# boguszjelinski/taxidispatcher

Hardware: AMD Instinct MI355X
Metric: NxN assignments/sec (higher is better)
Workload: dtype int32; 1 GPU; g1 N=16384: device cost write (4N^2 B) + exact assignment, total checked == optimum; n=16384, parallelism=single GPU

## Files before the change

taxidispatcher_amd/csrc/td_assign.hip:

```cpp
#include <dlfcn.h>
#include <limits.h>
#include <stdlib.h>

#include <type_traits>

#include "td_common.h"

using namespace td;

namespace {

template <typename CT>
struct Tr;
template <>
struct Tr<uint8_t> {
    using PT = int32_t;
    static constexpr int E = 16;
    static constexpr uint32_t SENT = 0xFFu;
    static constexpr int64_t LIMIT = 254;
    static constexpr int32_t BIG = 1 << 28;
    static constexpr int32_t KMAX = INT32_MAX;
};
template <>
struct Tr<uint16_t> {
// ... 100 lines not shown
int g_cgrid = 4;
int g_creg = 1;
int g_speculate = 1;
int g_sap8 = 1;
int g_psap8_batches = 1;
int g_psap8_grid = 64;
int g_warm_tie_div = 2;
int g_u16_redo_free = 64;
int g_wide_u16_n = 2048;
bool g_line = true;
int g_line_min_n = 2;
int g_psap_batches = 16;
int g_psap_min = 12;
int g_psap_cap = 4096;
int g_warm = 1;
int g_warm_div = 4;
int g_warm_theta = 2;
int g_warm_bits = 30;
int g_warm_groups = 32;
int g_warm_cut = 64;
int g_warm_min_range = 256;
int g_warm_minfree = 32;
int g_warm_min_n = 512;
int g_sapx = 1;
int g_sapx_min = 8;
int g_sapx_slim_chunks = INT_MAX;
int g_sapx_rows = 24;
int g_sap512 = 1;
int g_psap_worth = 4;
int g_bid0 = 1;
int g_defer_const = 1;
int g_shape = 1;
int g_shape_max_n = 1 << 20;
int g_narrow_price = 1;
long long g_np_plimit = NP_PLIMIT;
int g_fuse_t = 2;
int g_fuse_spec = 1;
int g_fused_rounds = 8;
int g_fuse_gen = 1;
int g_tick_rounds = 5;
int g_forest = 1;
int g_forest_min_n = 2048;
long long g_forest_w0 = 16;
long long g_forest_wx = 16;
int g_blocks = -1;
int g_blocks_min_n = 12288;
int g_zs_rounds = 4;
int g_zs_sep = 0;
int g_hop_passes = 2;
int g_hop_max_rows = HOP_FMAX;
int g_lazy_cc = 1;
int g_hop_global = 1;
int g_one_trip = 1;
int g_zs_global_rounds = 6;
int g_core = 1;
int g_core_k = 64;
int g_core_min_n = 8192;
int g_core_mode = 1;
double g_core_eps = 1.0;
int g_rand_test = 1;
int g_rand_div = 8192;
int g_rand_rounds = 48;
int g_rand_repeat = 1;
double g_rand_corr = 0.12;
int g_core_patience = 6;
int g_solver_eps = 0;
int g_eps_theta = 8;
long long g_eps0_mult = 4;
void read_tunables()
{
    static bool done = false;
    if (done) return;
    done = true;
    if (const char *e = getenv("TD_MAX_ROUNDS")) g_max_rounds = std::max(1, std::min(48, atoi(e)));
    if (const char *e = getenv("TD_TIE_EVICT")) g_tie_evict = atoi(e) != 0;
    if (const char *e = getenv("TD_LDS_ROUNDS")) g_lds_rounds = std::max(0, atoi(e));
    if (const char *e = getenv("TD_SAP8")) g_sap8 = atoi(e) != 0;
    if (const char *e = getenv("TD_ROW_LOOP")) g_row_loop = std::max(0, atoi(e));
    if (const char *e = getenv("TD_ROW_ROUNDS")) g_row_rounds = std::max(0, atoi(e));
    if (const char *e = getenv("TD_CGRID")) g_cgrid = std::max(1, atoi(e));
    if (const char *e = getenv("TD_CREG")) g_creg = atoi(e) != 0;
    if (const char *e = getenv("TD_PSAP")) g_psap_batches = std::max(0, std::min(64, atoi(e)));
    if (const char *e = getenv("TD_PSAP_MIN")) g_psap_min = std::max(1, atoi(e));
    if (const char *e = getenv("TD_PSAP_CAP")) g_psap_cap = std::max(0, atoi(e));
    if (const char *e = getenv("TD_SAP512")) g_sap512 = atoi(e) != 0;
    if (const char *e = getenv("TD_SAPX")) g_sapx = atoi(e) != 0;
    if (const char *e = getenv("TD_WARM")) g_warm = atoi(e) != 0;
    if (const char *e = getenv("TD_WARM_DIV")) g_warm_div = std::max(1, atoi(e));
    if (const char *e = getenv("TD_WARM_THETA")) g_warm_theta = std::max(2, atoi(e));
    if (const char *e = getenv("TD_WARM_BITS")) g_warm_bits = std::max(1, std::min(30, atoi(e)));
    if (const char *e = getenv("TD_WARM_GROUPS")) g_warm_groups = std::max(1, atoi(e));
    if (const char *e = getenv("TD_WARM_CUT")) g_warm_cut = std::max(0, atoi(e));
    if (const char *e = getenv("TD_WARM_MIN_RANGE")) g_warm_min_range = std::max(1, atoi(e));
    if (const char *e = getenv("TD_WARM_MINFREE")) g_warm_minfree = std::max(1, atoi(e));
    if (const char *e = getenv("TD_WARM_MIN_N")) g_warm_min_n = std::max(0, atoi(e));
    if (const char *e = getenv("TD_SAPX_MIN")) g_sapx_min = std::max(1, atoi(e));
    if (const char *e = getenv("TD_SAPX_SLIM")) g_sapx_slim_chunks = std::max(64, atoi(e));
    if (const char *e = getenv("TD_SAPX_ROWS")) g_sapx_rows = std::max(1, atoi(e));
    if (const char *e = getenv("TD_PSAP_WORTH")) g_psap_worth = std::max(1, atoi(e));
    if (const char *e = getenv("TD_SPECULATE")) g_speculate = atoi(e) != 0;
    if (const char *e = getenv("TD_LDS_GRID")) g_lds_grid = std::max(1, std::min(8, atoi(e)));
    if (const char *e = getenv("TD_NARROW_PRICE")) g_narrow_price = atoi(e) != 0;
    if (const char *e = getenv("TD_NP_PLIMIT")) g_np_plimit = std::max(1ll, std::min((long long)NP_PLIMIT, atoll(e)));
    if (const char *e = getenv("TD_FUSE_T")) g_fuse_t = std::max(0, std::min(2, atoi(e)));
    if (const char *e = getenv("TD_FUSE_SPEC")) g_fuse_spec = atoi(e) != 0;
    if (const char *e = getenv("TD_FUSED_ROUNDS")) g_fused_rounds = std::max(1, std::min(48, atoi(e)));
    if (const char *e = getenv("TD_FUSE_GEN")) g_fuse_gen = atoi(e) != 0;
    if (const char *e = getenv("TD_TICK_ROUNDS")) g_tick_rounds = std::max(1, std::min(48, atoi(e)));
    if (const char *e = getenv("TD_FOREST")) g_forest = atoi(e) != 0;
    if (const char *e = getenv("TD_FOREST_MIN_N")) g_forest_min_n = std::max(64, atoi(e));
    if (const char *e = getenv("TD_FOREST_W0")) g_forest_w0 = std::max(1ll, atoll(e));
    if (const char *e = getenv("TD_FOREST_WX")) g_forest_wx = std::max(0ll, atoll(e));
    if (const char *e = getenv("TD_SOLVER")) g_solver_eps = (strcmp(e, "eps") == 0);
    if (const char *e = getenv("TD_EPS0_MULT")) g_eps0_mult = std::max(0ll, atoll(e));
    if (const char *e = getenv("TD_EPS_THETA")) g_eps_theta = std::max(2, atoi(e));
    if (const char *e = getenv("TD_PSAP8")) g_psap8_batches = std::max(0, std::min(32, atoi(e)));
    if (const char *e = getenv("TD_DEFER_CONST")) g_defer_const = atoi(e) != 0;
    if (const char *e = getenv("TD_BID0")) g_bid0 = atoi(e) != 0;
    if (const char *e = getenv("TD_SHAPE")) g_shape = atoi(e) != 0;
    if (const char *e = getenv("TD_SHAPE_MAX_N")) g_shape_max_n = atoi(e);
    if (const char *e = getenv("TD_WIDE_U16_N")) g_wide_u16_n = std::max(0, atoi(e));
    if (const char *e = getenv("TD_U16_REDO_FREE")) g_u16_redo_free = std::max(0, atoi(e));
    if (const char *e = getenv("TD_WARM_TIE_DIV")) g_warm_tie_div = std::max(1, atoi(e));
    if (const char *e = getenv("TD_LINE")) g_line = atoi(e) != 0;
    if (const char *e = getenv("TD_LINE_MIN_N")) g_line_min_n = std::max(2, atoi(e));
    if (const char *e = getenv("TD_PSAP8_GRID")) g_psap8_grid = std::max(1, std::min(192, atoi(e)));
    if (const char *e = getenv("TD_CORE")) g_core = atoi(e) != 0;
    if (const char *e = getenv("TD_CORE_K")) g_core_k = std::max(2, std::min(200, atoi(e)));
    if (const char *e = getenv("TD_CORE_MIN_N")) g_core_min_n = std::max(256, atoi(e));
    if (const char *e = getenv("TD_CORE_MODE")) g_core_mode = atoi(e);
    if (const char *e = getenv("TD_CORE_EPS")) g_core_eps = atof(e);
    if (const char *e = getenv("TD_CORE_PATIENCE")) g_core_patience = std::max(1, atoi(e));
    if (const char *e = getenv("TD_RAND_TEST")) g_rand_test = atoi(e) != 0;
    if (const char *e = getenv("TD_RAND_DIV")) g_rand_div = std::max(1, atoi(e));
    if (const char *e = getenv("TD_RAND_ROUNDS")) g_rand_rounds = std::max(1, std::min(48, atoi(e)));
    if (const char *e = getenv("TD_RAND_CORR")) g_rand_corr = atof(e);
    if (const char *e = getenv("TD_RAND_REPEAT")) g_rand_repeat = std::max(1, atoi(e));
    if (const char *e = getenv("TD_BLOCKS")) g_blocks = std::max(-1, std::min(HOP_BMAX, atoi(e)));
    if (const char *e = getenv("TD_BLOCKS_MIN_N")) g_blocks_min_n = std::max(0, atoi(e));
    if (const char *e = getenv("TD_ZS_ROUNDS")) g_zs_rounds = std::max(0, std::min(32, atoi(e)));
    if (const char *e = getenv("TD_ZS_SEP")) g_zs_sep = atoi(e) != 0;
    if (const char *e = getenv("TD_HOP_PASSES")) g_hop_passes = std::max(0, std::min(8, atoi(e)));
    if (const char *e = getenv("TD_HOP_MAX_ROWS")) g_hop_max_rows = std::max(1, atoi(e));
    if (const char *e = getenv("TD_HOP_GLOBAL")) g_hop_global = atoi(e) != 0;
    if (const char *e = getenv("TD_ONE_TRIP")) g_one_trip = atoi(e) != 0;
    if (const char *e = getenv("TD_LAZY_CC")) g_lazy_cc = atoi(e) != 0;
    if (const char *e = getenv("TD_ZS_GLOBAL_ROUNDS")) g_zs_global_rounds = std::max(1, std::min(48, atoi(e)));
}

template <typename CT>
__device__ __forceinline__ void unpack(const uint4 &v, uint32_t *out);
template <>
__device__ __forceinline__ void unpack<uint8_t>(const uint4 &v, uint32_t *o)
{
    const uint32_t w[4] = {v.x, v.y, v.z, v.w};
#pragma unroll
    for (int k = 0; k < 4; k++) {
        o[4 * k + 0] = w[k] & 0xFFu;
        o[4 * k + 1] = (w[k] >> 8) & 0xFFu;
        o[4 * k + 2] = (w[k] >> 16) & 0xFFu;
        o[4 * k + 3] = w[k] >> 24;
    }
}
template <>
__device__ __forceinline__ void unpack<u8e>(const uint4 &v, uint32_t *o)
{
    const uint32_t w[4] = {v.x, v.y, v.z, v.w};
    const uint32_t esc = g_esc8;
#pragma unroll
    for (int k = 0; k < 4; k++) {
#pragma unroll
        for (int b = 0; b < 4; b++) {
            const uint32_t x = (w[k] >> (8 * b)) & 0xFFu;
            o[4 * k + b] = (x == U8E_ESC) ? esc : x;
        }
    }
}
template <>
__device__ __forceinline__ void unpack<uint16_t>(const uint4 &v, uint32_t *o)
{
    const uint32_t w[4] = {v.x, v.y, v.z, v.w};
#pragma unroll
    for (int k = 0; k < 4; k++) {
        o[2 * k + 0] = w[k] & 0xFFFFu;
        o[2 * k + 1] = w[k] >> 16;
    }
}
template <>
__device__ __forceinline__ void unpack<uint32_t>(const uint4 &v, uint32_t *o)
{
    o[0] = v.x;
    o[1] = v.y;
    o[2] = v.z;
    o[3] = v.w;
}
template <>
__device__ __forceinline__ void unpack<u32n>(const uint4 &v, uint32_t *o)
{
    o[0] = v.x;
// ... 2843 lines not shown
    using PT = typename Tr<CT>::PT;
    int rc;
    if ((rc = ensure(sv.esc, sizeof(unsigned long long) * 2 * (size_t)std::max(sv.nrows, 1)))) return rc;
    if ((rc = ensure(sv.hop, sizeof(HopCtl)))) return rc;
    if ((rc = ensure(sv.hoptab, sizeof(int) * (size_t)nb * HOP_FMAX * HOP_FMAX))) return rc;
    HopCtl *hc = (HopCtl *)sv.hop.p;
    int *frl = (int *)sv.list.p, *fcl = (int *)sv.pred.p;
    const int *ctl = (const int *)sv.misc.p;
    if (gate && nb != 1) return fail(TD_EINTERNAL, "a gated two-hop pass takes one block");
    k_hop_lists<<<nb, 1024, 0, c.stream>>>(rpb, ncols_blk, col_lo, (const int *)sv.r2c.p, (const int *)sv.owner.p, frl, fcl, hc, ctl,
                                           gate ? g_hop_max_rows : 0);
    if (raw) {
        if (!sv.d_cost || sv.n % 4) return fail(TD_EINVAL, "two-hop pass on the int32 matrix: no matrix, or n %% 4 != 0");
        k_hop_esc<CT, true><<<(sv.nrows + 3) / 4, 256, 0, c.stream>>>(sv.nrows, sv.n / 4, rpb, ncols_blk, col_lo, g_hop_max_rows,
                                                                      (const CT *)sv.d_cost, (const PT *)sv.price.p, (const int *)sv.r2c.p, fcl,
                                                                      hc, (unsigned long long *)sv.esc.p, ctl, (const int32_t *)sv.rowmin.p);
        k_hop_table<CT, true><<<nb * HOP_FMAX, 256, 0, c.stream>>>(sv.n, sv.nrows, sv.row0, sv.n / 4, rpb, ncols_blk, col_lo, g_hop_max_rows,
                                                                   window_zero ? 1 : 0, (const CT *)sv.d_cost, (const PT *)sv.price.p,
                                                                   (const int *)sv.owner.p, frl, hc, (const unsigned long long *)sv.esc.p,
                                                                   (int *)sv.hoptab.p, ctl, (const int32_t *)sv.rowmin.p);
    } else {
    k_hop_esc<CT><<<(sv.nrows + 3) / 4, 256, 0, c.stream>>>(sv.nrows, sv.nchunks, rpb, ncols_blk, col_lo, g_hop_max_rows, (const CT *)sv.cc.p,
                                                            (const PT *)sv.price.p, (const int *)sv.r2c.p, fcl, hc,
                                                            (unsigned long long *)sv.esc.p, ctl);
    k_hop_table<CT><<<nb * HOP_FMAX, 256, 0, c.stream>>>(sv.n, sv.nrows, sv.row0, sv.nchunks, rpb, ncols_blk, col_lo, g_hop_max_rows,
                                                         window_zero ? 1 : 0, (const CT *)sv.cc.p, (const PT *)sv.price.p,
                                                         (const int *)sv.owner.p, frl, hc, (const unsigned long long *)sv.esc.p,
                                                         (int *)sv.hoptab.p, ctl);
    }
    k_hop_match<PT><<<nb, HOP_FMAX, sizeof(uint32_t) * (size_t)((rpb + 31) / 32), c.stream>>>(
        sv.nrows, sv.row0, rpb, ncols_blk, col_lo, g_hop_max_rows, (PT *)sv.price.p, (int *)sv.owner.p, (int *)sv.r2c.p, ob, frl, fcl, hc,
        (const int *)sv.hoptab.p, (int *)sv.misc.p);
    TD_HIP(hipGetLastError());
    return TD_OK;
}

template <typename CT>
int sv_begin_t(Solver &sv);

int sv_phase_a(Solver &sv, int hop_passes)
{
    Ctx &c = ctx();
    const int n = sv.n, nrows = sv.nrows;
    const int rpb = n / sv.zs_V, nb = nrows / rpb;
    const int col_lo = (sv.row0 / rpb) * rpb, col_hi = col_lo + nb * rpb;
    int rc;
    if ((rc = ensure(sv.ob, (size_t)sv.npad + 64))) return rc;
    if (!sv.ob_clear) TD_HIP(hipMemsetAsync(sv.ob.p, 0, (size_t)sv.npad, c.stream));
    sv.ob_clear = false;
    ProfScope ps(TD_K_BID);
    int *ctl = (int *)sv.misc.p;
    const int ga = (col_hi - col_lo + 255) / 256;
    unsigned long long *bid = (unsigned long long *)sv.bid.p;
    auto assign = [&]() {
        k_zs_assign<<<ga, 256, 0, c.stream>>>(col_lo, col_hi, nrows, sv.row0, bid, (int32_t *)sv.price.p, (int *)sv.owner.p, (int *)sv.r2c.p,
                                              (uint8_t *)sv.ob.p, ctl);
    };
    if (sv.zs_round0) {
        if (!sv.began && (rc = sv_begin_t<uint8_t>(sv))) return rc;
        k_zs_bid<<<std::min(nrows, c.n_cu * 16), 256, 0, c.stream>>>(nrows, sv.row0, sv.nchunks, rpb, (const uint8_t *)sv.cc.p,
                                                                     (const uint8_t *)sv.ob.p, (const int *)sv.r2c.p, bid, ctl, 0, 0);
        sv.zs_round0 = false;
    }
    assign();
    for (int r = 1; r <= g_zs_rounds; r++) {
        k_zs_bid<<<std::min(nrows, c.n_cu * 16), 256, 0, c.stream>>>(nrows, sv.row0, sv.nchunks, rpb, (const uint8_t *)sv.cc.p,
                                                                     (const uint8_t *)sv.ob.p, (const int *)sv.r2c.p, bid, ctl, r, g_tie_evict);
        assign();
    }
    TD_HIP(hipGetLastError());
    for (int p = 0; p < hop_passes; p++)
        if ((rc = sv_hop_t<uint8_t>(sv, rpb, rpb, col_lo, nb, true, (uint8_t *)sv.ob.p))) return rc;
    if (getenv("TD_DEBUG") && hop_passes > 0) {
        HopCtl h;
        TD_HIP(hipMemcpyAsync(&h, sv.hop.p, sizeof(h), hipMemcpyDeviceToHost, c.stream));
        TD_HIP(hipStreamSynchronize(c.stream));
        fprintf(stderr, "[td] phase A: %d blocks of %d rows, %d local rounds; free rows / columns per block before the last two-hop pass:", nb, rpb, g_zs_rounds);
        for (int b = 0; b < nb; b++) fprintf(stderr, " %d/%d", h.nfr[b], h.nfc[b]);
        fprintf(stderr, " | matched %d, left %d\n", h.matched, h.left);
    }
    sv.zs_done = false;
    sv.bid0_done = false;
    sv.state_ready = true;
    return TD_OK;
}

template <typename CT>
int sv_begin_t(Solver &sv)
{
    Ctx &c = ctx();
    using PT = typename Tr<CT>::PT;
    const PT padkey = (PT)(Tr<CT>::BIG << 1) | (PT)1;
    k_init_state<PT><<<(std::max(sv.npad, (int)CTL_WORDS) + 255) / 256, 256, 0, c.stream>>>(
        sv.n, sv.npad, sv.nrows, (PT *)sv.price.p, padkey, (int *)sv.owner.p, (int *)sv.r2c.p,
        (unsigned long long *)sv.bid.p, (int *)sv.misc.p, sv.defer_const ? (const int *)sv.rconst.p : nullptr, sv.probe, 0, nullptr,
        g_one_trip ? (unsigned long long *)((char *)sv.misc.p + FIN_OFF) : nullptr);
    if (!g_one_trip) TD_HIP(hipMemsetAsync((char *)sv.misc.p + FIN_OFF, 0, 16, c.stream));
    TD_HIP(hipGetLastError());
    sv.began = true;
    return TD_OK;
}

template <typename CT>
int sv_bid_t(Solver &sv, int r, unsigned long long *keys)
{
    Ctx &c = ctx();
    using PT = typename Tr<CT>::PT;
    const int n = sv.n, nrows = sv.nrows;
    if (nrows == 0) return TD_OK;
    const size_t lds_prices = (size_t)sv.npad * sizeof(PT);
    const bool can_lds = lds_prices <= 128 * 1024 && n >= 2048 && nrows >= 1024;
    const int tie_evict = (r >= 1) ? g_tie_evict : 0;
    ProfScope ps(TD_K_BID);
    int *tied = (r == 0) ? (int *)sv.misc.p + CTL_TIED : nullptr;
    const bool sparse = sv.state_ready;
    if (can_lds && r < g_lds_rounds && !sparse) {
        if (lds_prices > 48 * 1024)
            (void)hipFuncSetAttribute((const void *)k_bid<CT, true>, hipFuncAttributeMaxDynamicSharedMemorySize, (int)lds_prices);
        const int grid = std::min((nrows + 15) / 16, c.n_cu * g_lds_grid);
        k_bid<CT, true><<<grid, 1024, lds_prices, c.stream>>>(n, nrows, sv.row0, sv.nchunks, (const CT *)sv.cc.p, (const PT *)sv.price.p,
                                                              (const int *)sv.r2c.p, keys, (const int *)sv.misc.p, r, tie_evict, 1, 0, tied);
    } else if (r >= g_row_rounds || sparse) {
        k_bid_row<CT><<<(r < g_row_loop && !sparse) ? nrows : std::min(nrows, c.n_cu * 8), 256, 0, c.stream>>>(n, nrows, sv.row0, sv.nchunks, (const CT *)sv.cc.p, (const PT *)sv.price.p,
                                                   (const int *)sv.r2c.p, keys, (const int *)sv.misc.p, r, tie_evict);
    } else {
// ... 1255 lines not shown
__global__ void k_state_import(int n, int world, int rps, int words, int own_rank, const int32_t *__restrict__ all,
                               int *__restrict__ owner, int32_t *__restrict__ pk, int *__restrict__ cmask, long long *__restrict__ summary)
{
    const int t = blockIdx.x * blockDim.x + threadIdx.x;
    if (t == 0) {
        long long fit = 1, ran = 1, left = 0, nconst = 0, range = 0;
        for (int r = 0; r < world; r++) {
            const int32_t *h = all + (size_t)r * words;
            fit = fit && h[0];
            ran = ran && h[1];
            left += h[2] >= 0 ? h[2] : n;
            nconst += h[3];
            const long long rg = (long long)(((unsigned long long)(uint32_t)h[5] << 32) | (uint32_t)h[4]);
            range = rg > range ? rg : range;
        }
        summary[0] = fit;
        summary[1] = ran;
        summary[2] = left;
        summary[3] = nconst;
        summary[4] = range;
        summary[5] = all[6];
    }
    if (t < n) {
        const int r = t / rps, k = t - r * rps;
        const int32_t *seg = all + (size_t)r * words;
        if (r != own_rank) {
            const int o = seg[16 + k];
            owner[t] = o;
            pk[t] = (pk[t] & ~1) | (o >= 0 ? 1 : 0);
        }
        cmask[t] = seg[16 + rps + k];
    }
}
}

extern "C" {
int td_shard_state_export(td_shard *s, int rows_per_shard, int fits, int32_t *seg)
{
    TD_REQUIRE_INIT();
    Ctx &c = ctx();
    if (!s || !seg || rows_per_shard < s->nrows) return fail(TD_EINVAL, "td_shard_state_export: bad arguments");
    if (!is_device_ptr(seg)) return fail(TD_EINVAL, "td_shard_state_export: the segment must be device memory");
    const bool ran = s->state_ready && s->bpc == 1 && s->zs_V > 0;
    int col_lo = 0;
    if (ran) col_lo = (s->row0 / (s->n / s->zs_V)) * (s->n / s->zs_V);
    ProfScope ps(TD_K_ASSIGN);
    k_state_export<<<(std::max(rows_per_shard, 16) + 255) / 256, 256, 0, c.stream>>>(
        s->nrows, rows_per_shard, col_lo, fits ? 1 : 0, ran ? 1 : 0, (const int *)s->owner.p, (const int *)s->rconst.p,
        ran ? (const HopCtl *)s->hop.p : nullptr, (const int *)s->misc.p, seg);
    TD_HIP(hipGetLastError());
    return TD_OK;
}

int td_shard_state_import(td_shard *s, int world, int rank, int rows_per_shard, const int32_t *all, int64_t *summary5)
{
    TD_REQUIRE_INIT();
    Ctx &c = ctx();
    if (!s || !all || !summary5 || world < 1 || rank < 0 || rank >= world) return fail(TD_EINVAL, "td_shard_state_import: bad arguments");
    if (!is_device_ptr(all)) return fail(TD_EINVAL, "td_shard_state_import: the segments must be device memory");
    if ((long long)rows_per_shard * world < s->n) return fail(TD_EINVAL, "td_shard_state_import: rows_per_shard * world < n");
    int rc;
    if ((rc = ensure(s->cmask, sizeof(int) * (size_t)(s->n + 16)))) return rc;
    long long *sum_dev = (long long *)((char *)s->misc.p + 2048);
    const int words = 16 + 2 * rows_per_shard;
    {
        ProfScope ps(TD_K_ASSIGN);
        k_state_import<<<(s->n + 255) / 256, 256, 0, c.stream>>>(s->n, world, rows_per_shard, words, rank, all, (int *)s->owner.p,
                                                            (int32_t *)s->price.p, (int *)s->cmask.p, sum_dev);
    }
    TD_HIP(hipGetLastError());
    TD_HIP(hipMemcpyAsync(c.pinned, sum_dev, 6 * sizeof(long long), hipMemcpyDeviceToHost, c.stream));
    TD_HIP(hipStreamSynchronize(c.stream));
    for (int k = 0; k < 6; k++) summary5[k] = ((const long long *)c.pinned)[k];
    s->have_cmask = true;
    s->defer_const = g_defer_const && !g_solver_eps;
    return TD_OK;
}

int td_shard_range(td_shard *s, int64_t *range)
{
    TD_REQUIRE_INIT();
    if (!s || !range) return fail(TD_EINVAL, "null argument");
    *range = s->range > 0 ? s->range : std::max<int64_t>(0, s->fit_bound);
    return TD_OK;
}

int td_shard_begin(td_shard *s, int64_t global_range)
{
    TD_REQUIRE_INIT();
    if (!s) return fail(TD_EINVAL, "null shard");
    const int64_t range = global_range >= 0 ? global_range : (s->range > 0 ? s->range : std::max<int64_t>(0, s->fit_bound));
    if ((double)(range + 1) * (double)(s->n + 1) >= 4.0e12)
        return fail(TD_ERANGE, "row cost range %lld with n=%d overflows the packed bid key (price < 2^43)", (long long)range, s->n);
    int rc = TD_OK;
    if (!s->bid0_done && !s->state_ready) TD_DISPATCH(*s, sv_begin_t, *s);
    return rc;
}

int td_shard_keys_len(td_shard *s) { return s ? s->npad : 0; }

namespace {
int shard_bid_round(td_shard *s, int round, unsigned long long *keys)
{
    int rc = TD_OK;
    if ((rc = sv_complete_cc(*s))) return rc;
    if (round == 0 && s->bid0_done) {
        const size_t bytes = sizeof(unsigned long long) * (size_t)s->npad;
        TD_HIP(hipMemcpyAsync(keys, s->bid.p, bytes, hipMemcpyDeviceToDevice, ctx().stream));
        TD_HIP(hipMemsetAsync(s->bid.p, 0, bytes, ctx().stream));
        return TD_OK;
    }
    TD_DISPATCH(*s, sv_bid_t, *s, round, keys);
    return rc;
}
}

int td_shard_bid(td_shard *s, int round, uint64_t *keys)
{
    TD_REQUIRE_INIT();
    if (!s || !keys) return fail(TD_EINVAL, "null argument");
    if (!is_device_ptr(keys)) return fail(TD_EINVAL, "bid keys must be device memory");
    return shard_bid_round(s, round, (unsigned long long *)keys);
}

int td_shard_apply(td_shard *s, int round, uint64_t *keys)
{
// ... 293 lines not shown
```

taxidispatcher_amd/csrc/td_blocks.h:

```cpp


struct HopCtl {
    int nfr[HOP_BMAX], nfc[HOP_BMAX];
    int left;
    int matched;
    int pad[2];
};

__device__ __forceinline__ uint32_t zs_zero_bytes(uint32_t w)
{
    return ~(((w & 0x7F7F7F7Fu) + 0x7F7F7F7Fu) | w | 0x7F7F7F7Fu);
}

__global__ __launch_bounds__(256) void k_zs_bid(int nrows, int row0, int nchunks, int rpb, const uint8_t *__restrict__ cc,
                                                const uint8_t *__restrict__ ob, const int *__restrict__ r2c,
                                                unsigned long long *__restrict__ bid, const int *__restrict__ ctl, int round,
                                                int tie_evict)
{
    __shared__ int s_best[4];
    if (ctl[CTL_FLAG]) return;
    const int tid = threadIdx.x, lane = tid & 63, w = tid >> 6;
    const int cpb = rpb >> 4;
    const size_t pitch = (size_t)nchunks * 16;
    for (int lrow = blockIdx.x; lrow < nrows; lrow += gridDim.x) {
        if (r2c[lrow] != -1) continue;
        const int row = row0 + lrow;
        const int c0 = (row / rpb) * cpb;
        const uint32_t hsh = ((uint32_t)row + 1u) * 0x9E3779B1u + (uint32_t)round * 0x85EBCA6Bu;
        const int rot = (int)(((uint64_t)(hsh ^ (hsh >> 15)) * (uint64_t)cpb) >> 32);
        const uint8_t *rp = cc + (size_t)lrow * pitch;
        int best = INT_MAX;
        for (int t = tid; t < cpb; t += 256) {
            int ch = t + rot;
            if (ch >= cpb) ch -= cpb;
            ch += c0;
            const uint4 cv = *reinterpret_cast<const uint4 *>(rp + (size_t)ch * 16);
            const uint4 ov = *reinterpret_cast<const uint4 *>(ob + (size_t)ch * 16);
            const uint32_t cw[4] = {cv.x, cv.y, cv.z, cv.w}, ow[4] = {ov.x, ov.y, ov.z, ov.w};
#pragma unroll
            for (int k = 0; k < 4; k++) {
                const uint32_t z = zs_zero_bytes(cw[k]);
                if (!z) continue;
                const uint32_t zf = z & zs_zero_bytes(ow[k]);
                const uint32_t pick = zf ? zf : z;
                const int cand = (zf ? 0 : (1 << 24)) | (t * 16 + k * 4 + (__builtin_ctz(pick) >> 3));
                best = min(best, cand);
            }
        }
#pragma unroll
        for (int o = 32; o > 0; o >>= 1) best = min(best, __shfl_xor(best, o));
        if (lane == 0) s_best[w] = best;
        __syncthreads();
        if (tid == 0) {
            best = min(min(s_best[0], s_best[1]), min(s_best[2], s_best[3]));
            if (best != INT_MAX) {
                const bool owned = (best >> 24) != 0;
                const int pos = best & 0xFFFFFF;
                int ch = (pos >> 4) + rot;
                if (ch >= cpb) ch -= cpb;
                const int j = (c0 + ch) * 16 + (pos & 15);
                if (!owned || tie_evict) atomicMax(&bid[j], (unsigned long long)(row + 1));
            }
        }
        __syncthreads();
    }
}

__global__ __launch_bounds__(256) void k_zs_assign(int col_lo, int col_hi, int nrows, int row0, unsigned long long *__restrict__ bid,
                                                   int32_t *__restrict__ pk, int *__restrict__ owner, int *__restrict__ r2c,
                                                   uint8_t *__restrict__ ob, const int *__restrict__ ctl)
{
    if (ctl[CTL_FLAG]) return;
    const int j = col_lo + blockIdx.x * blockDim.x + threadIdx.x;
    if (j >= col_hi) return;
    const unsigned long long k = bid[j];
    if (!k) return;
    const int row = (int)(k & ((1ull << ROW_BITS) - 1)) - 1;
    const int old = owner[j];
    if (old >= row0 && old < row0 + nrows) r2c[old - row0] = -1;
    owner[j] = row;
    if (row >= row0 && row < row0 + nrows) r2c[row - row0] = j;
    pk[j] = 1;
    ob[j] = 1;
    bid[j] = 0ull;
}

__global__ __launch_bounds__(1024) void k_hop_lists(int rpb, int ncols_blk, int col_lo, const int *__restrict__ r2c,
                                                    const int *__restrict__ owner, int *__restrict__ frl, int *__restrict__ fcl,
                                                    HopCtl *__restrict__ hc, const int *__restrict__ ctl, int gate_max = 0)
{
    if (ctl[CTL_FLAG]) return;
    const int lb = blockIdx.x;
    if (gate_max > 0) {
        __shared__ int s_go;
        if (threadIdx.x == 0) {
            const int left = hc->left;
            s_go = left > 0 && left <= gate_max;
        }
        __syncthreads();
        if (!s_go) {
            if (threadIdx.x == 0) hc->nfr[lb] = 0, hc->nfc[lb] = 0;
            return;
        }
    }
    const int nfr = build_free_list(rpb, r2c + (size_t)lb * rpb, frl + (size_t)lb * rpb, -1);
    const int nfc = build_free_list(ncols_blk, owner + col_lo + (size_t)lb * ncols_blk, fcl + (size_t)lb * ncols_blk, -1);
    if (threadIdx.x == 0) {
        hc->nfr[lb] = nfr;
        hc->nfc[lb] = nfc;
        if (lb == 0) hc->left = 0, hc->matched = 0;
    }
}

template <typename CT, bool RAW = false>
__global__ __launch_bounds__(256) void k_hop_esc(int nrows, int nchunks, int rpb, int ncols_blk, int col_lo, int max_rows,
                                                 const CT *__restrict__ cc, const typename Tr<CT>::PT *__restrict__ pk,
                                                 const int *__restrict__ r2c, const int *__restrict__ fcl,
                                                 const HopCtl *__restrict__ hc, unsigned long long *__restrict__ esc,
                                                 const int *__restrict__ ctl, const int32_t *__restrict__ rowmin = nullptr)
{
    using PT = typename Tr<CT>::PT;
    if (ctl[CTL_FLAG]) return;
    const int lane = threadIdx.x & 63;
    const int lrow = blockIdx.x * 4 + (threadIdx.x >> 6);
    if (lrow >= nrows) return;
// ... 189 lines not shown
    s_usedc[tid] = 0;
    __syncthreads();
    const int *fr = frl + (size_t)lb * rpb, *fc = fcl + (size_t)lb * ncols_blk;
    const int blk_row0 = row0 + lb * rpb;
    const int my_fc = tid < nc ? fc[tid] : 0;
    int done = 0;
    int r_nx = tid < nc ? tab[((size_t)lb * HOP_FMAX + 0) * HOP_FMAX + tid] : -1;
    int i_nx = blk_row0 + fr[0];
    for (int a = 0; a < na; a++) {
        const int r = r_nx, i_g = i_nx;
        if (a + 1 < na) {
            r_nx = tid < nc ? tab[((size_t)lb * HOP_FMAX + a + 1) * HOP_FMAX + tid] : -1;
            i_nx = blk_row0 + fr[a + 1];
        }
        const uint32_t hsh = ((uint32_t)i_g + 1u) * 0x9E3779B1u;
        const int st = nc ? (int)(((uint64_t)(hsh ^ (hsh >> 15)) * (uint64_t)nc) >> 32) : 0;
        int key = INT_MAX;
        if (r >= 0 && !s_usedc[tid]) {
            const int rb = r - blk_row0;
            if (!((s_usedr[rb >> 5] >> (rb & 31)) & 1u)) {
                int t = tid - st;
                t += t < 0 ? nc : 0;
                key = t;
            }
        }
        int best = key;
#pragma unroll
        for (int o = 32; o > 0; o >>= 1) best = min(best, __shfl_xor(best, o));
        if (lane == 0) s_key[a & 1][w] = best;
        __syncthreads();
        best = min(s_key[a & 1][0], s_key[a & 1][1]);
        if (best != INT_MAX && key == best) {
            const int rl = r - row0, il = i_g - row0;
            const int j = r2c[rl], jp = col_lo + lb * ncols_blk + my_fc;
            r2c[il] = j;
            owner[j] = i_g;
            r2c[rl] = jp;
            owner[jp] = r;
            pk[jp] = pk[jp] | (PT)1;
            if (ob) ob[jp] = 1;
            s_usedc[tid] = 1;
            const int rb = r - blk_row0;
            atomicOr(&s_usedr[rb >> 5], 1u << (rb & 31));
        }
        if (best != INT_MAX) done++;
        __syncthreads();
    }
    if (tid == 0) {
        atomicAdd(&hc->left, nfr - done);
        atomicAdd(&hc->matched, done);
    }
}

__global__ void k_zs_owned_bits(int n, const int *__restrict__ owner, int32_t *__restrict__ pk)
{
    const int j = blockIdx.x * blockDim.x + threadIdx.x;
    if (j < n) pk[j] = (pk[j] & ~1) | (owner[j] >= 0 ? 1 : 0);
}
```

Before: 27.67 million assignments/s.

## Fuse late zero-slack bidding rounds and two-hop passes into one per-block kernel

Adds k_block_tail, a 1024-thread kernel that runs one workgroup per diagonal block. Each workgroup keeps the block's r2c, owner and ob state in LDS and runs the remaining zero-slack bid/assign rounds plus the two-hop augmentation passes inside the kernel, using LDS atomics instead of global bid arrays. This replaces many small kernel launches (bid, assign, hop list/escape/table/match) with one launch, so launch overhead and global round-trips should drop. The cost is that each block now runs in a single workgroup with a large LDS footprint, which gives limited parallelism when few blocks exist. The unused k_zs_owned_bits kernel is removed and a parameter is renamed.

After: 26.45 million assignments/s. 0.956x the previous value.

```diff
diff --git a/taxidispatcher_amd/csrc/td_assign.hip b/taxidispatcher_amd/csrc/td_assign.hip
--- a/taxidispatcher_amd/csrc/td_assign.hip
+++ b/taxidispatcher_amd/csrc/td_assign.hip
@@ -176,6 +176,8 @@
 int g_lazy_cc = 1;
 int g_hop_global = 1;
 int g_one_trip = 1;
+int g_block_tail = 1;
+int g_block_tail_from = 3;
 int g_zs_global_rounds = 6;
 int g_core = 1;
 int g_core_k = 64;
@@ -269,6 +271,8 @@
     if (const char *e = getenv("TD_HOP_GLOBAL")) g_hop_global = atoi(e) != 0;
     if (const char *e = getenv("TD_ONE_TRIP")) g_one_trip = atoi(e) != 0;
     if (const char *e = getenv("TD_LAZY_CC")) g_lazy_cc = atoi(e) != 0;
+    if (const char *e = getenv("TD_BLOCK_TAIL")) g_block_tail = atoi(e) != 0;
+    if (const char *e = getenv("TD_BLOCK_TAIL_FROM")) g_block_tail_from = std::max(1, std::min(33, atoi(e)));
     if (const char *e = getenv("TD_ZS_GLOBAL_ROUNDS")) g_zs_global_rounds = std::max(1, std::min(48, atoi(e)));
 }
 
@@ -3218,9 +3222,18 @@
     int *ctl = (int *)sv.misc.p;
     const int ga = (col_hi - col_lo + 255) / 256;
     unsigned long long *bid = (unsigned long long *)sv.bid.p;
+    const int tail_from = std::max(1, std::min(g_block_tail_from, g_zs_rounds + 1));
+    const size_t tail_lds = bt_lds_bytes(rpb);
+    const bool tail = g_block_tail && nb > 0 && rpb <= 32768 && tail_lds <= (size_t)156 * 1024 && (tail_from <= g_zs_rounds || hop_passes > 0);
+    HopCtl *hc_zero = nullptr;
+    if (tail) {
+        if ((rc = ensure(sv.esc, sizeof(unsigned long long) * 2 * (size_t)std::max(nrows, 1)))) return rc;
+        if ((rc = ensure(sv.hop, sizeof(HopCtl)))) return rc;
+        if (hop_passes > 0) hc_zero = (HopCtl *)sv.hop.p;
+    }
     auto assign = [&]() {
         k_zs_assign<<<ga, 256, 0, c.stream>>>(col_lo, col_hi, nrows, sv.row0, bid, (int32_t *)sv.price.p, (int *)sv.owner.p, (int *)sv.r2c.p,
-                                              (uint8_t *)sv.ob.p, ctl);
+                                              (uint8_t *)sv.ob.p, ctl, hc_zero);
     };
     if (sv.zs_round0) {
         if (!sv.began && (rc = sv_begin_t<uint8_t>(sv))) return rc;
@@ -3229,14 +3242,26 @@
         sv.zs_round0 = false;
     }
     assign();
-    for (int r = 1; r <= g_zs_rounds; r++) {
+    for (int r = 1; r <= (tail ? tail_from - 1 : g_zs_rounds); r++) {
         k_zs_bid<<<std::min(nrows, c.n_cu * 16), 256, 0, c.stream>>>(nrows, sv.row0, sv.nchunks, rpb, (const uint8_t *)sv.cc.p,
                                                                      (const uint8_t *)sv.ob.p, (const int *)sv.r2c.p, bid, ctl, r, g_tie_evict);
         assign();
     }
     TD_HIP(hipGetLastError());
-    for (int p = 0; p < hop_passes; p++)
-        if ((rc = sv_hop_t<uint8_t>(sv, rpb, rpb, col_lo, nb, true, (uint8_t *)sv.ob.p))) return rc;
+    if (tail) {
+        static size_t lds_set = 0;
+        if (tail_lds > lds_set) {
+            TD_HIP(hipFuncSetAttribute((const void *)k_block_tail<int32_t>, hipFuncAttributeMaxDynamicSharedMemorySize, (int)tail_lds));
+            lds_set = tail_lds;
+        }
+        k_block_tail<int32_t><<<nb, BT_THREADS, tail_lds, c.stream>>>(sv.row0, sv.nchunks, rpb, col_lo, (const uint8_t *)sv.cc.p, (int32_t *)sv.price.p,
+                                                                      (int *)sv.owner.p, (int *)sv.r2c.p, (uint8_t *)sv.ob.p, (uint32_t *)sv.esc.p,
+                                                                      (HopCtl *)sv.hop.p, ctl, tail_from, g_zs_rounds, g_tie_evict, hop_passes,
+                                                                      g_hop_max_rows);
+        TD_HIP(hipGetLastError());
+    } else
+        for (int p = 0; p < hop_passes; p++)
+            if ((rc = sv_hop_t<uint8_t>(sv, rpb, rpb, col_lo, nb, true, (uint8_t *)sv.ob.p))) return rc;
     if (getenv("TD_DEBUG") && hop_passes > 0) {
         HopCtl h;
         TD_HIP(hipMemcpyAsync(&h, sv.hop.p, sizeof(h), hipMemcpyDeviceToHost, c.stream));
@@ -4598,11 +4623,11 @@
     return TD_OK;
 }
 
-int td_shard_state_import(td_shard *s, int world, int rank, int rows_per_shard, const int32_t *all, int64_t *summary5)
+int td_shard_state_import(td_shard *s, int world, int rank, int rows_per_shard, const int32_t *all, int64_t *summary6)
 {
     TD_REQUIRE_INIT();
     Ctx &c = ctx();
-    if (!s || !all || !summary5 || world < 1 || rank < 0 || rank >= world) return fail(TD_EINVAL, "td_shard_state_import: bad arguments");
+    if (!s || !all || !summary6 || world < 1 || rank < 0 || rank >= world) return fail(TD_EINVAL, "td_shard_state_import: bad arguments");
     if (!is_device_ptr(all)) return fail(TD_EINVAL, "td_shard_state_import: the segments must be device memory");
     if ((long long)rows_per_shard * world < s->n) return fail(TD_EINVAL, "td_shard_state_import: rows_per_shard * world < n");
     int rc;
@@ -4617,7 +4642,7 @@
     TD_HIP(hipGetLastError());
     TD_HIP(hipMemcpyAsync(c.pinned, sum_dev, 6 * sizeof(long long), hipMemcpyDeviceToHost, c.stream));
     TD_HIP(hipStreamSynchronize(c.stream));
-    for (int k = 0; k < 6; k++) summary5[k] = ((const long long *)c.pinned)[k];
+    for (int k = 0; k < 6; k++) summary6[k] = ((const long long *)c.pinned)[k];
     s->have_cmask = true;
     s->defer_const = g_defer_const && !g_solver_eps;
     return TD_OK;
diff --git a/taxidispatcher_amd/csrc/td_blocks.h b/taxidispatcher_amd/csrc/td_blocks.h
--- a/taxidispatcher_amd/csrc/td_blocks.h
+++ b/taxidispatcher_amd/csrc/td_blocks.h
@@ -68,9 +68,11 @@
 
 __global__ __launch_bounds__(256) void k_zs_assign(int col_lo, int col_hi, int nrows, int row0, unsigned long long *__restrict__ bid,
                                                    int32_t *__restrict__ pk, int *__restrict__ owner, int *__restrict__ r2c,
-                                                   uint8_t *__restrict__ ob, const int *__restrict__ ctl)
+                                                   uint8_t *__restrict__ ob, const int *__restrict__ ctl,
+                                                   HopCtl *__restrict__ hc_zero = nullptr)
 {
     if (ctl[CTL_FLAG]) return;
+    if (hc_zero && blockIdx.x == 0 && threadIdx.x == 0) hc_zero->left = 0, hc_zero->matched = 0;
     const int j = col_lo + blockIdx.x * blockDim.x + threadIdx.x;
     if (j >= col_hi) return;
     const unsigned long long k = bid[j];
@@ -366,8 +368,341 @@
     }
 }
 
-__global__ void k_zs_owned_bits(int n, const int *__restrict__ owner, int32_t *__restrict__ pk)
-{
-    const int j = blockIdx.x * blockDim.x + threadIdx.x;
-    if (j < n) pk[j] = (pk[j] & ~1) | (owner[j] >= 0 ? 1 : 0);
-}
+constexpr int BT_THREADS = 1024, BT_WAVES = BT_THREADS / 64;
+constexpr int BT_ER = 4;
+
+__host__ __device__ inline size_t bt_round16(size_t x) { return (x + 15) & ~(size_t)15; }
+__host__ __device__ inline size_t bt_union_bytes(int rpb)
+{
+    const size_t a = (size_t)rpb * 4;
+    const size_t b = bt_round16(rpb) + (size_t)HOP_FMAX * HOP_FMAX * 2 + (size_t)BT_WAVES * HOP_FMAX * 4;
+    return bt_round16(a > b ? a : b);
+}
+__host__ __device__ inline size_t bt_bits_bytes(int rpb) { return bt_round16((size_t)((rpb + 31) / 32) * 4); }
+__host__ __device__ inline size_t bt_lds_bytes(int rpb)
+{
+    return bt_round16(rpb) + 2 * bt_round16((size_t)rpb * 4) + bt_round16((size_t)rpb * 2) + 2 * bt_bits_bytes(rpb) + bt_union_bytes(rpb);
+}
+
+__device__ __forceinline__ void bt_wave_sync()
+{
+    __builtin_amdgcn_fence(__ATOMIC_ACQ_REL, "wavefront");
+    __builtin_amdgcn_wave_barrier();
+}
+
+template <typename PT>
+__global__ __launch_bounds__(BT_THREADS) void k_block_tail(int row0, int nchunks, int rpb, int col_lo, const uint8_t *__restrict__ cc,
+                                                           PT *__restrict__ pk, int *__restrict__ owner, int *__restrict__ r2c,
+                                                           uint8_t *__restrict__ ob, uint32_t *__restrict__ esc, HopCtl *__restrict__ hc,
+                                                           const int *__restrict__ ctl, int round_from, int round_to, int tie_evict,
+                                                           int hop_passes, int max_rows)
+{
+    extern __shared__ __attribute__((aligned(16))) unsigned char bt_smem[];
+    __shared__ int s_fr[HOP_FMAX], s_fc[HOP_FMAX];
+    __shared__ int s_scan[BT_WAVES];
+    __shared__ int s_cnt, s_tot;
+    __shared__ uint32_t s_wesc[BT_WAVES][BT_ER][4];
+    if (ctl[CTL_FLAG]) return;
+    const int tid = threadIdx.x, lane = tid & 63, w = tid >> 6, lb = blockIdx.x;
+    const int cb = col_lo + lb * rpb;
+    const int lrow0 = lb * rpb;
+    const int blk_row0 = row0 + lrow0;
+    const int cpb = rpb >> 4;
+    const size_t pitch = (size_t)nchunks * 16;
+    const uint8_t *cblk = cc + (size_t)lrow0 * pitch + cb;
+
+    unsigned char *sp = bt_smem;
+    uint8_t *s_ob = sp;
+    sp += bt_round16(rpb);
+    int *s_r2c = reinterpret_cast<int *>(sp);
+    sp += bt_round16((size_t)rpb * 4);
+    int *s_own = reinterpret_cast<int *>(sp);
+    sp += bt_round16((size_t)rpb * 4);
+    uint16_t *s_list = reinterpret_cast<uint16_t *>(sp);
+    sp += bt_round16((size_t)rpb * 2);
+    uint32_t *s_need = reinterpret_cast<uint32_t *>(sp);
+    sp += bt_bits_bytes(rpb);
+    uint32_t *s_usedr = reinterpret_cast<uint32_t *>(sp);
+    sp += bt_bits_bytes(rpb);
+    uint32_t *s_bid = reinterpret_cast<uint32_t *>(sp);
+    uint8_t *s_colb = sp;
+    uint16_t *s_tab = reinterpret_cast<uint16_t *>(sp + bt_round16(rpb));
+    int *s_trow = reinterpret_cast<int *>(sp + bt_round16(rpb) + (size_t)HOP_FMAX * HOP_FMAX * 2);
+    const int nbits = (rpb + 31) / 32;
+
+    for (int i = tid; i < rpb; i += BT_THREADS) {
+        const int v = r2c[lrow0 + i], o = owner[cb + i];
+        s_r2c[i] = v < 0 ? v : ((unsigned)(v - cb) < (unsigned)rpb ? v - cb : -3);
+        s_own[i] = (unsigned)(o - blk_row0) < (unsigned)rpb ? o - blk_row0 : -1;
+        s_ob[i] = ob[cb + i];
+        s_bid[i] = 0u;
+    }
+    if (tid < BT_WAVES * BT_ER * 4) (&s_wesc[0][0][0])[tid] = 0u;
+    __syncthreads();
+
+    for (int round = round_from; round <= round_to; round++) {
+        if (tid == 0) s_cnt = 0;
+        __syncthreads();
+        for (int i = tid; i < rpb; i += BT_THREADS)
+            if (s_r2c[i] == -1) s_list[atomicAdd(&s_cnt, 1)] = (uint16_t)i;
+        __syncthreads();
+        const int nf = s_cnt;
+        for (int k = w; k < nf; k += 2 * BT_WAVES) {
+            const int ia = s_list[k];
+            const bool two = k + BT_WAVES < nf;
+            const int ib = two ? s_list[k + BT_WAVES] : ia;
+            const uint32_t ha = ((uint32_t)(blk_row0 + ia) + 1u) * 0x9E3779B1u + (uint32_t)round * 0x85EBCA6Bu;
+            const uint32_t hb = ((uint32_t)(blk_row0 + ib) + 1u) * 0x9E3779B1u + (uint32_t)round * 0x85EBCA6Bu;
+            const int rota = (int)(((uint64_t)(ha ^ (ha >> 15)) * (uint64_t)cpb) >> 32);
+            const int rotb = (int)(((uint64_t)(hb ^ (hb >> 15)) * (uint64_t)cpb) >> 32);
+            const uint8_t *rpa = cblk + (size_t)ia * pitch, *rpb_ = cblk + (size_t)ib * pitch;
+            int besta = INT_MAX, bestb = INT_MAX;
+            for (int t = lane; t < cpb; t += 64) {
+                int cha = t + rota, chb = t + rotb;
+                if (cha >= cpb) cha -= cpb;
+                if (chb >= cpb) chb -= cpb;
+                const uint4 cva = *reinterpret_cast<const uint4 *>(rpa + (size_t)cha * 16);
+                const uint4 cvb = *reinterpret_cast<const uint4 *>(rpb_ + (size_t)chb * 16);
+                const uint4 ova = *reinterpret_cast<const uint4 *>(s_ob + (size_t)cha * 16);
+                const uint4 ovb = *reinterpret_cast<const uint4 *>(s_ob + (size_t)chb * 16);
+                const uint32_t cwa[4] = {cva.x, cva.y, cva.z, cva.w}, owa[4] = {ova.x, ova.y, ova.z, ova.w};
+                const uint32_t cwb[4] = {cvb.x, cvb.y, cvb.z, cvb.w}, owb[4] = {ovb.x, ovb.y, ovb.z, ovb.w};
+#pragma unroll
+                for (int q = 0; q < 4; q++) {
+                    const uint32_t za = zs_zero_bytes(cwa[q]);
+                    if (za) {
+                        const uint32_t zf = za & zs_zero_bytes(owa[q]);
+                        const uint32_t pick = zf ? zf : za;
+                        besta = min(besta, (zf ? 0 : (1 << 24)) | (t * 16 + q * 4 + (__builtin_ctz(pick) >> 3)));
+                    }
+                    const uint32_t zb = zs_zero_bytes(cwb[q]);
+                    if (zb) {
+                        const uint32_t zf = zb & zs_zero_bytes(owb[q]);
+                        const uint32_t pick = zf ? zf : zb;
+                        bestb = min(bestb, (zf ? 0 : (1 << 24)) | (t * 16 + q * 4 + (__builtin_ctz(pick) >> 3)));
+                    }
+                }
+            }
+#pragma unroll
+            for (int o = 32; o > 0; o >>= 1) {
+                besta = min(besta, __shfl_xor(besta, o));
+                bestb = min(bestb, __shfl_xor(bestb, o));
+            }
+            if (lane < 2 && (lane == 0 || two)) {
+                const int best = lane ? bestb : besta, rot = lane ? rotb : rota, i = lane ? ib : ia;
+                if (best != INT_MAX) {
+                    const bool owned = (best >> 24) != 0;
+                    const int pos = best & 0xFFFFFF;
+                    int ch = (pos >> 4) + rot;
+                    if (ch >= cpb) ch -= cpb;
+                    if (!owned || tie_evict) atomicMax(&s_bid[ch * 16 + (pos & 15)], (uint32_t)(i + 1));
+                }
+            }
+        }
+        __syncthreads();
+        for (int j = tid; j < rpb; j += BT_THREADS) {
+            const uint32_t key = s_bid[j];
+            if (!key) continue;
+            s_bid[j] = 0u;
+            const int i = (int)key - 1, old = s_own[j];
+            if (old >= 0) s_r2c[old] = -1, r2c[lrow0 + old] = -1;
+            s_own[j] = i, owner[cb + j] = blk_row0 + i;
+            s_r2c[i] = j, r2c[lrow0 + i] = cb + j;
+            pk[cb + j] = (PT)1;
+            s_ob[j] = 1, ob[cb + j] = 1;
+        }
+        __syncthreads();
+    }
+
+    int last_left = 0, last_matched = 0;
+    for (int p = 0; p < hop_passes; p++) {
+        const int per = (rpb + BT_THREADS - 1) / BT_THREADS;
+        const int lo = min(rpb, tid * per), hi = min(rpb, lo + per);
+        int cnt = 0;
+        for (int i = lo; i < hi; i++) cnt += (s_r2c[i] == -1 ? 1 : 0) + (s_own[i] == -1 ? 1 << 16 : 0);
+        int incl = cnt;
+#pragma unroll
+        for (int o = 1; o < 64; o <<= 1) {
+            const int v = __shfl_up(incl, o);
+            if (lane >= o) incl += v;
+        }
+        if (lane == 63) s_scan[w] = incl;
+        __syncthreads();
+        int base = 0;
+        for (int k = 0; k < w; k++) base += s_scan[k];
+        if (tid == BT_THREADS - 1) s_tot = base + incl;
+        int pr = (base + incl - cnt) & 0xFFFF, pc = (base + incl - cnt) >> 16;
+        for (int i = lo; i < hi; i++) {
+            if (s_r2c[i] == -1) {
+                if (pr < HOP_FMAX) s_fr[pr] = i;
+                pr++;
+            }
+            if (s_own[i] == -1) {
+                if (pc < HOP_FMAX) s_fc[pc] = i;
+                pc++;
+            }
+        }
+        for (int i = tid; i < (int)(bt_round16(rpb) / 4); i += BT_THREADS) reinterpret_cast<uint32_t *>(s_colb)[i] = 0xFFFFFFFFu;
+        for (int i = tid; i < nbits; i += BT_THREADS) s_need[i] = 0u, s_usedr[i] = 0u;
+        if (tid == 0) s_cnt = 0;
+        __syncthreads();
+        const int nfr = s_tot & 0xFFFF, nfc = s_tot >> 16;
+        if (tid == 0) hc->nfr[lb] = nfr, hc->nfc[lb] = nfc;
+        if (nfr == 0 || nfr > max_rows) {
+            last_left = nfr, last_matched = 0;
+            break;
+        }
+        const int na = min(nfr, HOP_FMAX), nc = min(nfc, HOP_FMAX);
+        if (tid < nc) s_colb[s_fc[tid]] = (uint8_t)tid;
+        for (int a = w; a < na; a += BT_WAVES) {
+            const uint8_t *rp = cblk + (size_t)s_fr[a] * pitch;
+            for (int t = lane; t < cpb; t += 64) {
+                const uint4 cv = *reinterpret_cast<const uint4 *>(rp + (size_t)t * 16);
+                const uint32_t cw[4] = {cv.x, cv.y, cv.z, cv.w};
+#pragma unroll
+                for (int q = 0; q < 4; q++) {
+                    uint32_t z = zs_zero_bytes(cw[q]);
+                    while (z) {
+                        const int rb = s_own[t * 16 + q * 4 + (__builtin_ctz(z) >> 3)];
+                        z &= z - 1;
+                        if (rb >= 0) atomicOr(&s_need[rb >> 5], 1u << (rb & 31));
+                    }
+                }
+            }
+        }
+        __syncthreads();
+        for (int i = tid; i < rpb; i += BT_THREADS)
+            if ((s_need[i >> 5] >> (i & 31)) & 1u) s_list[atomicAdd(&s_cnt, 1)] = (uint16_t)i;
+        __syncthreads();
+        const int nn = s_cnt;
+        for (int k = w; k < nn; k += BT_ER * BT_WAVES) {
+            int rr[BT_ER];
+            const uint8_t *rp[BT_ER];
+#pragma unroll
+            for (int e = 0; e < BT_ER; e++) {
+                rr[e] = k + e * BT_WAVES < nn ? (int)s_list[k + e * BT_WAVES] : -1;
+                rp[e] = cblk + (size_t)(rr[e] < 0 ? (int)s_list[k] : rr[e]) * pitch;
+            }
+            for (int t0 = 0; t0 < cpb; t0 += 128) {
+                uint4 cv[2][BT_ER];
+#pragma unroll
+                for (int u = 0; u < 2; u++) {
+                    const int t = min(t0 + u * 64 + lane, cpb - 1);
+#pragma unroll
+                    for (int e = 0; e < BT_ER; e++) cv[u][e] = *reinterpret_cast<const uint4 *>(rp[e] + (size_t)t * 16);
+                }
+#pragma unroll
+                for (int u = 0; u < 2; u++) {
+                    const int t = t0 + u * 64 + lane;
+                    if (t >= cpb) continue;
+                    const uint4 mv = *reinterpret_cast<const uint4 *>(s_colb + (size_t)t * 16);
+                    const uint32_t mw[4] = {mv.x, mv.y, mv.z, mv.w};
+#pragma unroll
+                    for (int e = 0; e < BT_ER; e++) {
+                        if (rr[e] < 0) continue;
+                        const uint32_t cw[4] = {cv[u][e].x, cv[u][e].y, cv[u][e].z, cv[u][e].w};
+#pragma unroll
+                        for (int q = 0; q < 4; q++) {
+                            uint32_t z = zs_zero_bytes(cw[q]) & zs_zero_bytes(mw[q] & 0x80808080u);
+                            while (z) {
+                                const uint32_t b = (mw[q] >> (__builtin_ctz(z) & 24)) & 0xFFu;
+                                z &= z - 1;
+                                atomicOr(&s_wesc[w][e][b >> 5], 1u << (b & 31));
+                            }
+                        }
+                    }
+                }
+            }
+            bt_wave_sync();
+            int myr = -1;
+#pragma unroll
+            for (int e = 0; e < BT_ER; e++) myr = (lane >> 2) == e ? rr[e] : myr;
+            if (myr >= 0) esc[(size_t)(lrow0 + myr) * 4 + (lane & 3)] = atomicExch(&s_wesc[w][lane >> 2][lane & 3], 0u);
+            bt_wave_sync();
+        }
+        __syncthreads();
+        for (int a = w; a < na; a += BT_WAVES) {
+            int *trow = s_trow + w * HOP_FMAX;
+            trow[lane] = INT_MAX, trow[lane + 64] = INT_MAX;
+            bt_wave_sync();
+            const uint8_t *rp = cblk + (size_t)s_fr[a] * pitch;
+            for (int t = lane; t < cpb; t += 64) {
+                const uint4 cv = *reinterpret_cast<const uint4 *>(rp + (size_t)t * 16);
+                const uint32_t cw[4] = {cv.x, cv.y, cv.z, cv.w};
+#pragma unroll
+                for (int q = 0; q < 4; q++) {
+                    uint32_t z = zs_zero_bytes(cw[q]);
+                    while (z) {
+                        const int rb = s_own[t * 16 + q * 4 + (__builtin_ctz(z) >> 3)];
+                        z &= z - 1;
+                        if (rb < 0) continue;
+                        const uint4 m = *reinterpret_cast<const uint4 *>(esc + (size_t)(lrow0 + rb) * 4);
+                        const uint32_t mw[4] = {m.x, m.y, m.z, m.w};
+#pragma unroll
+                        for (int u = 0; u < 4; u++) {
+                            uint32_t bits = mw[u];
+                            while (bits) {
+                                atomicMin(&trow[u * 32 + __builtin_ctz(bits)], rb);
+                                bits &= bits - 1;
+                            }
+                        }
+                    }
+                }
+            }
+            bt_wave_sync();
+            const int v0 = trow[lane], v1 = trow[lane + 64];
+            s_tab[a * HOP_FMAX + lane] = v0 == INT_MAX ? (uint16_t)0xFFFF : (uint16_t)v0;
+            s_tab[a * HOP_FMAX + lane + 64] = v1 == INT_MAX ? (uint16_t)0xFFFF : (uint16_t)v1;
+            bt_wave_sync();
+        }
+        __syncthreads();
+        if (w == 0) {
+            const int fc0 = lane < nc ? s_fc[lane] : 0, fc1 = lane + 64 < nc ? s_fc[lane + 64] : 0;
+            bool usedc0 = false, usedc1 = false;
+            volatile uint32_t *usedr = s_usedr;
+            int done = 0;
+            for (int a = 0; a < na; a++) {
+                const int i = s_fr[a];
+                const uint32_t hsh = ((uint32_t)(blk_row0 + i) + 1u) * 0x9E3779B1u;
+                const int st = nc ? (int)(((uint64_t)(hsh ^ (hsh >> 15)) * (uint64_t)nc) >> 32) : 0;
+                const int r0 = lane < nc ? (int)s_tab[a * HOP_FMAX + lane] : 0xFFFF;
+                const int r1 = lane + 64 < nc ? (int)s_tab[a * HOP_FMAX + lane + 64] : 0xFFFF;
+                int key0 = INT_MAX, key1 = INT_MAX;
+                if (r0 != 0xFFFF && !usedc0 && !((usedr[r0 >> 5] >> (r0 & 31)) & 1u)) {
+                    const int t = lane - st;
+                    key0 = t + (t < 0 ? nc : 0);
+                }
+                if (r1 != 0xFFFF && !usedc1 && !((usedr[r1 >> 5] >> (r1 & 31)) & 1u)) {
+                    const int t = lane + 64 - st;
+                    key1 = t + (t < 0 ? nc : 0);
+                }
+                const int key = min(key0, key1);
+                int best = key;
+#pragma unroll
+                for (int o = 32; o > 0; o >>= 1) best = min(best, __shfl_xor(best, o));
+                if (best != INT_MAX && key == best) {
+                    const bool second = key0 != best;
+                    const int rb = second ? r1 : r0, jp = second ? fc1 : fc0;
+                    const int j = s_r2c[rb];
+                    s_r2c[i] = j, r2c[lrow0 + i] = cb + j;
+                    s_own[j] = i, owner[cb + j] = blk_row0 + i;
+                    s_r2c[rb] = jp, r2c[lrow0 + rb] = cb + jp;
+                    s_own[jp] = rb, owner[cb + jp] = blk_row0 + rb;
+                    pk[cb + jp] = pk[cb + jp] | (PT)1;
+                    s_ob[jp] = 1, ob[cb + jp] = 1;
+                    if (second) usedc1 = true;
+                    else usedc0 = true;
+                    atomicOr(&s_usedr[rb >> 5], 1u << (rb & 31));
+                }
+                if (best != INT_MAX) done++;
+                bt_wave_sync();
+            }
+            last_left = nfr - done, last_matched = done;
+        }
+        __syncthreads();
+    }
+    if (hop_passes > 0 && tid == 0) {
+        atomicAdd(&hc->left, last_left);
+        atomicAdd(&hc->matched, last_matched);
+    }
+}
```
